# wanzysky/SlenderObjDet

Hardware: AMD Instinct MI355X
Metric: training img/sec FCOS R50-FPN 1333x800 (higher is better)
Workload: dtype bf16; 1 GPU; FCOS R50-FPN (FCOSV2, giou, center-sampling 1.5), fwd+bwd+SGD, synthetic 1333x800 padded to 800x1344 (BASELINE.json configs[1]); global_batch=16, parallelism=dp1

## Files before the change

### slenderobjdet_amd/csrc/conv_args.h

```cpp
#pragma once
#include "common.h"
#include "../../include/slender_hip.h"
#include <stdlib.h>

namespace sodconv {

enum { MODE_FWD = 0, MODE_DGRAD = 1 };
enum {
  F_BIAS = 1, F_RELU = 2, F_RES = 4, F_RES_UP2 = 8, F_MASK = 16,
  F_WBITS = 64,
  F_MASKBITS = 128,
  F_GNSTATS = 32,
  F_REVERSE = 1024,
  F_RES_EVEN = 512,
};
constexpr int MAXLEV = SOD_CONV_MAX_LEVELS;

struct LevelGeo {
  const void* src;
  void* dst;
  const void* res;
  const void* mask;
  void* bits;
  float* gn_sum;
// ... 46 lines not shown
template <int LPR>
__device__ __forceinline__ void gn_acc_finish(GnAcc& g, uint32_t pa, uint32_t pb, uint32_t P, const FastDiv& div_hw, float* sums, int G, int grp,
                                              bool qok, int lane) {
  if (pa >= P) return;
  if (pb >= P) pb = P - 1;
  const int na = (int)fd_div(pa, div_hw), nb = (int)fd_div(pb, div_hw);
  if (na == nb) {
    float s = (g.n >= 0) ? g.s : 0.f, ss = (g.n >= 0) ? g.ss : 0.f;
#pragma unroll
    for (int o = LPR; o < 64; o <<= 1) { s += __shfl_xor(s, o, 64); ss += __shfl_xor(ss, o, 64); }
    if (lane < LPR && qok) {
      atomicAdd(sums + ((size_t)na * G + grp) * 2, s);
      atomicAdd(sums + ((size_t)na * G + grp) * 2 + 1, ss);
    }
  } else if (qok) {
    gn_acc_flush(g, sums, G, grp);
  }
}

enum ConvTile { TILE_16x256, TILE_64x256, TILE_64x256_K32, TILE_128x128, TILE_128x128_K32 };
int launch_conv128(const ConvArgs& a, int mode, bool out_f32, ConvTile tile, bool generic, hipStream_t st, int* variant);

bool conv256_supported(const ConvArgs& a, int mode);
int launch_conv256(const ConvArgs& a, int mode, bool out_f32, int max_pt_tiles, hipStream_t st);

bool pw_supported(const ConvArgs& a, int mode, bool out_f32, int cus);
int launch_pw(const ConvArgs& a, int mode, hipStream_t st);

bool ws3_supported(const ConvArgs& a, int mode, bool out_f32, int cus, bool any_size);
int launch_ws3(const ConvArgs& a, int mode, hipStream_t st);

struct WLevel {
  const void* dy;
  const void* x;
  uint32_t dy_bytes, x_bytes;
  int Hx, Wx, Ho, Wo, P;
  int v0;
  int dy_img_stride, x_img_stride;
  FastDiv div_hw, div_w;
};

struct WgradArgs {
  WLevel lev[MAXLEV];
  int nlev;
  float* dw;
  const float* qscale;
  int dbg_plain_store;
// ... 31 lines not shown
```

### slenderobjdet_amd/csrc/conv_dispatch.hip

```cpp
#include "conv_args.h"
#include <stdlib.h>
#include <atomic>
#include <algorithm>

using namespace sodconv;

int device_cus() {
  static const int cus = [] {
    int dev = 0, n = 0;
    if (hipGetDevice(&dev) != hipSuccess || hipDeviceGetAttribute(&n, hipDeviceAttributeMultiprocessorCount, dev) != hipSuccess || n <= 0) n = 256;
    return n;
  }();
  return cus;
}

namespace {

thread_local int g_last_variant = 0;
thread_local int g_conv_reverse = 0;

struct ConvKnobs {
  int conv256 = -1;
  int pw = -1;
  int ws3 = -1;
  int wgrad256 = 1;
  int wgrad9 = 1;
  int wgrad9_min_kt = 24;
  int wgrad_variant = -1;
};
ConvKnobs& knobs() {
  const auto env = [](const char* name, int dflt) { const char* e = getenv(name); return e ? atoi(e) : dflt; };
  static ConvKnobs k = [&] {
    ConvKnobs k0;
    k0.wgrad256 = env("SOD_WGRAD256", k0.wgrad256);
    k0.wgrad9 = env("SOD_WGRAD9", k0.wgrad9);
    k0.wgrad9_min_kt = env("SOD_WGRAD9_MIN_KT", k0.wgrad9_min_kt);
    return k0;
  }();
  if (k.conv256 < 0) k.conv256 = env("SOD_CONV256", 1);
  if (k.pw < 0) k.pw = env("SOD_CONV_PW", 1);
  if (k.ws3 < 0) k.ws3 = env("SOD_CONV_WS3", 1);
  return k;
}

struct ConvProf {
  hipEvent_t* ev = nullptr;
  int* variant = nullptr;
  int* mode = nullptr;
  float* frac = nullptr;
  int cap = 0;
  std::atomic<int> n{0};
  std::atomic<int> on{0};
};
ConvProf g_prof;
thread_local int g_prof_depth = 0;
inline int prof_begin(hipStream_t st) {
  ConvProf& p = g_prof;
  if (!p.on.load(std::memory_order_relaxed) || g_prof_depth) return -1;
  const int i = p.n.fetch_add(1);
  if (i >= p.cap) { p.n.store(p.cap); return -1; }
  (void)hipEventRecord(p.ev[2 * i], st);
  return i;
// ... 20 lines not shown
  if (a.cwin) {
    if (generic || a.nlev != 1 || (a.Nout & 127)) return SOD_EARG;
    return conv128(TILE_128x128);
  }
  const ConvKnobs& k = knobs();
  const int cus = device_cus();
  if (k.pw && pw_supported(a, mode, out_f32, cus)) {
    g_last_variant = 7001;
    return timed(st, 7001, 1.f, mode, [&] { return launch_pw(a, mode, st); });
  }
  if (k.ws3 && ws3_supported(a, mode, out_f32, cus, k.ws3 == 2)) {
    g_last_variant = 7003;
    return timed(st, 7003, 1.f, mode, [&] { return launch_ws3(a, mode, st); });
  }
  bool any_start = false;
  for (int l = 0; l < a.nlev; ++l) any_start |= a.lev[l].pstart != 0;
  if (k.conv256 && !any_start && !(a.flags & (F_WBITS | F_MASKBITS)) && conv256_supported(a, mode)) {
    const int nq = (a.Nout + 255) / 256;
    long long pt256 = 0;
    for (int l = 0; l < a.nlev; ++l) pt256 += (a.lev[l].P + 255) / 256;
    const long long b256 = pt256 * nq;
    const auto conv256 = [&](int max_pt_tiles, float frac) {
      g_last_variant = 256;
      return timed(st, 256, frac, mode, [&] { return launch_conv256(a, mode, out_f32, max_pt_tiles, st); });
    };
    if (k.conv256 == 2) return conv256(0, 1.f);
    constexpr int min_rounds = 1, min_k = 1024;
    if (a.Nout >= 256 && ((a.Nout & 255) == 0 || a.Nout >= 512) && a.Kred >= min_k && b256 >= (long long)min_rounds * cus) {
      const long long full = b256 / cus * cus, rem = b256 - full;
      if (rem == 0 || rem * 2 >= (long long)cus || (full / nq) * nq != full) return conv256(0, 1.f);
      int main_pt = (int)(full / nq);
      long long ptot = 0;
      for (int l = 0; l < a.nlev; ++l) ptot += a.lev[l].P;
      int rc = conv256(main_pt, (float)((double)main_pt * 256.0 / (double)ptot));
      if (rc) return rc;
      ConvArgs tail = a;
      for (int l = 0; l < tail.nlev; ++l) {
        const int tl = (tail.lev[l].P + 255) / 256;
        if (main_pt >= tl) { tail.lev[l].pstart = tail.lev[l].P; main_pt -= tl; }
        else { tail.lev[l].pstart = main_pt * 256; main_pt = 0; }
      }
      ++g_prof_depth;
      rc = dispatch_conv(tail, mode, out_f32, st);
      --g_prof_depth;
      g_last_variant = 256;
      return rc;
    }
// ... 419 lines not shown
  return SOD_OK;
}

extern "C" int sod_conv_set_wgrad_variant(int variant) {
  if (variant < -1) return SOD_EARG;
  knobs().wgrad_variant = variant;
  return SOD_OK;
}

extern "C" int sod_conv_set_ws3(int mode) {
  if (mode < -1 || mode > 2) return SOD_EARG;
  knobs().ws3 = mode;
  return SOD_OK;
}

extern "C" int sod_conv_set_pw(int on) {
  if (on < -1 || on > 1) return SOD_EARG;
  knobs().pw = on;
  return SOD_OK;
}

extern "C" int sod_conv_set_tile256(int mode) {
  if (mode < -1 || mode > 2) return SOD_EARG;
  knobs().conv256 = mode;
  return SOD_OK;
}
```

### slenderobjdet_amd/csrc/conv_igemm256.hip

```cpp
#include "conv_args.h"
#include <stdlib.h>
#include <type_traits>

namespace sodconv {
namespace {

constexpr int ROWB = 128;
constexpr int UNIT = 128 * ROWB;
constexpr int BUF = 4 * UNIT;
constexpr int LDS_BYTES = 2 * BUF;
constexpr int E16_PITCH = 256;

template <int SA, int SB, int KS>
__device__ __forceinline__ void mma_half(f32x4_t (&acc)[8][4], const bf16x8_t (&af)[4][2], const bf16x8_t (&bf)[2][2]) {
#pragma unroll
  for (int i = 0; i < 4; ++i)
#pragma unroll
    for (int j = 0; j < 2; ++j)
      acc[SA * 4 + i][SB * 2 + j] = __builtin_amdgcn_mfma_f32_16x16x32_bf16(af[i][KS], bf[j][KS], acc[SA * 4 + i][SB * 2 + j], 0, 0, 0);
}

#define SOD256_SB __builtin_amdgcn_sched_barrier(0);
#define SOD256_PHASE(SA, SB, BFR, STAGE)                                  \
  asm volatile("s_waitcnt vmcnt(6)" ::: "memory");                        \
  __builtin_amdgcn_s_barrier();                                           \
  asm volatile("s_waitcnt lgkmcnt(0)" ::: "memory");                      \
  SOD256_SB                                                               \
  __builtin_amdgcn_s_setprio(1);                                          \
  mma_half<SA, SB, 0>(acc, af, BFR);                                      \
  SOD256_SB                                                               \
  STAGE;                                                                  \
  SOD256_SB                                                               \
  mma_half<SA, SB, 1>(acc, af, BFR);                                      \
  __builtin_amdgcn_s_setprio(0);                                          \
  __builtin_amdgcn_s_barrier();

template <int MODE, bool OUT_F32>
__global__ __launch_bounds__(512, 2) void conv_igemm256_kernel(const ConvArgs a) {
  extern __shared__ __attribute__((aligned(16))) char smem[];
  const int tid = threadIdx.x, lane = tid & 63;
  const int wave = __builtin_amdgcn_readfirstlane(tid >> 6);
  const int wr = wave >> 2, wc = wave & 3;
  uint32_t bid = xcd_remap(blockIdx.x, gridDim.x);
  if (a.flags & F_REVERSE) bid = gridDim.x - 1 - bid;
  const int qt = bid % a.nq_tiles;
  int pt = bid / a.nq_tiles;
  int lv = 0;
#pragma unroll
  for (int i = 1; i < MAXLEV; ++i)
    if (i < a.nlev && pt >= a.lev[i].tile0) lv = i;
  const LevelGeo& g = a.lev[lv];
  pt -= g.tile0;
  const int q0 = qt * 256, p0 = pt * 256;
  const int gP = g.P, gHs = g.Hs, gWs = g.Ws;
  const int T = a.T;

  auto wrsrc = __builtin_amdgcn_make_buffer_rsrc(const_cast<void*>(a.w), 0, a.w_bytes, 0x00020000);
  auto xrsrc = __builtin_amdgcn_make_buffer_rsrc(const_cast<void*>(g.src), 0, g.src_bytes, 0x00020000);

  const int srow = lane >> 3, spos = lane & 7;
  const int sswz = (lane >> 4) | ((wave & 1) << 2);
  const int schunk = spos ^ sswz;
  uint32_t wbase[2][2], rowbase[2][2], tapmask[2][2];
#pragma unroll
  for (int u = 0; u < 2; ++u)
#pragma unroll
    for (int j = 0; j < 2; ++j) {
      const int L = (j * 8 + wave) * 8 + srow;
      const int q = q0 + (L >> 6) * 128 + u * 64 + (L & 63);
      wbase[u][j] = (q < a.Nout) ? ((uint32_t)q * (uint32_t)a.Kred + (uint32_t)schunk * 8u) * 2u : SOD_OOB;
    }
  const uint32_t rs_mul = a.div_rs.mul, rs_shr = a.div_rs.shr, rs_d = a.div_rs.d;
  const int aCred = a.Cred;
  const bool pitched = a.Cpitch < a.Cred;
  auto stage_a = [&](int u, int kt) {
    char* dst = smem + (kt & 1) * BUF + u * UNIT + wave * 1024;
    const bool live = kt < T;
    const uint32_t kk = live ? (uint32_t)kt : 0u;
    const uint32_t cc = (__umulhi(kk, rs_mul) + kk) >> rs_shr;
    const uint32_t woff = ((kk - cc * rs_d) * (uint32_t)aCred + cc * 64u) * 2u;
    const uint32_t dead = live ? 0u : SOD_OOB;
#pragma unroll
    for (int j = 0; j < 2; ++j) {
      const uint32_t voff = (wbase[u][j] + woff) | dead;
      __builtin_amdgcn_raw_ptr_buffer_load_lds(wrsrc, SOD_LDS(dst + j * 8192), 16, voff, 0, 0, 0);
    }
  };
  stage_a(0, 0); stage_a(1, 0);
#pragma unroll
  for (int u = 0; u < 2; ++u)
#pragma unroll
    for (int j = 0; j < 2; ++j) {
      const int L = (j * 8 + wave) * 8 + srow;
      const uint32_t p = (uint32_t)(p0 + (L >> 5) * 64 + u * 32 + (L & 31));
      uint32_t m = 0, rb = 0;
      if (p < (uint32_t)gP) {
        const uint32_t n = fd_div(p, g.div_hw);
        const uint32_t rem = p - n * g.div_hw.d;
        const uint32_t ph = fd_div(rem, g.div_w);
        const uint32_t pw = rem - ph * g.div_w.d;
        int xh, xw;
        if (MODE == MODE_FWD) { xh = (int)ph * a.stride - a.pad; xw = (int)pw * a.stride - a.pad; }
        else                  { xh = (int)ph + a.pad;            xw = (int)pw + a.pad; }
        rb = (n * (uint32_t)g.src_img_stride + ((uint32_t)xh * (uint32_t)gWs + (uint32_t)xw) * (uint32_t)a.Cpitch + (uint32_t)schunk * 8u) * 2u;
        uint32_t colbits = 0;
        for (int s2 = 0; s2 < a.S; ++s2) {
          const int w = (MODE == MODE_FWD) ? xw + s2 * a.dil : xw - s2 * a.dil;
          colbits |= (uint32_t)((unsigned)w < (unsigned)gWs) << s2;
        }
        for (int r = 0; r < a.R; ++r) {
          const int h = (MODE == MODE_FWD) ? xh + r * a.dil : xh - r * a.dil;
          if ((unsigned)h < (unsigned)gHs) m |= colbits << (r * a.S);
        }
      }
      rowbase[u][j] = rb; tapmask[u][j] = m;
    }
  const int tap_sign = (MODE == MODE_FWD) ? 1 : -1;

  const uint32_t s_mul = a.div_s.mul, s_shr = a.div_s.shr;
  const int aS = a.S, row_step = a.dil * gWs * a.Cpitch * 2 * tap_sign, col_step = a.dil * a.Cpitch * 2 * tap_sign;

  auto stage_b = [&](int u, int kt) {
    char* dst = smem + (kt & 1) * BUF + (2 + u) * UNIT + wave * 1024;
    const bool live = kt < T;
    const uint32_t kk = live ? (uint32_t)kt : 0u;
    const uint32_t cc = (__umulhi(kk, rs_mul) + kk) >> rs_shr;
    const uint32_t tap = kk - cc * rs_d;
    const int c0 = (int)cc * 128;
    const int r = (int)((__umulhi(tap, s_mul) + tap) >> s_shr);
    const int s2 = (int)tap - r * aS;
    const uint32_t tapoff = (uint32_t)(r * row_step + s2 * col_step + c0);
    const uint32_t tbit = live ? tap : 31u;
    const bool cin = !pitched || ((int)cc * 64 + schunk * 8 < a.Cpitch);
#pragma unroll
    for (int j = 0; j < 2; ++j) {
      const uint32_t voff = (((tapmask[u][j] >> tbit) & 1u) && cin) ? rowbase[u][j] + tapoff : SOD_OOB;
      __builtin_amdgcn_raw_ptr_buffer_load_lds(xrsrc, SOD_LDS(dst + j * 8192), 16, voff, 0, 0, 0);
    }
  };

  const int fr = lane & 15, fg = lane >> 4;
  uint32_t aoff[4], boff[2];
#pragma unroll
  for (int i = 0; i < 4; ++i) {
    const int L = wr * 64 + i * 16 + fr;
    aoff[i] = L * ROWB + ((fg ^ ((L >> 1) & 7)) << 4);
  }
#pragma unroll
  for (int j = 0; j < 2; ++j) {
    const int L = wc * 32 + j * 16 + fr;
    boff[j] = 2 * UNIT + L * ROWB + ((fg ^ ((L >> 1) & 7)) << 4);
  }

  f32x4_t acc[8][4];
#pragma unroll
  for (int i = 0; i < 8; ++i)
#pragma unroll
    for (int j = 0; j < 4; ++j) acc[i][j] = f32x4_t{0.f, 0.f, 0.f, 0.f};
  bf16x8_t af[4][2], bf0[2][2], bf1[2][2];

  auto read_a = [&](const char* buf, int s) {
#pragma unroll
    for (int i = 0; i < 4; ++i)
#pragma unroll
      for (int ks = 0; ks < 2; ++ks) af[i][ks] = *reinterpret_cast<const bf16x8_t*>(buf + s * UNIT + (aoff[i] ^ (ks << 6)));
  };
  auto read_b = [&](const char* buf, int s, bf16x8_t (&bfr)[2][2]) {
#pragma unroll
    for (int j = 0; j < 2; ++j)
#pragma unroll
      for (int ks = 0; ks < 2; ++ks) bfr[j][ks] = *reinterpret_cast<const bf16x8_t*>(buf + s * UNIT + (boff[j] ^ (ks << 6)));
  };

  stage_b(0, 0); stage_b(1, 0);
  stage_a(0, 1); stage_b(0, 1);
  asm volatile("s_waitcnt vmcnt(4)" ::: "memory");
  __builtin_amdgcn_s_barrier();
  if (wr == 1) __builtin_amdgcn_s_barrier();

  for (int k = 0; k < T; ++k) {
    const char* cur = smem + (k & 1) * BUF;
    read_b(cur, 0, bf0);
    read_a(cur, 0);
    SOD256_PHASE(0, 0, bf0, stage_b(1, k + 1))
    read_b(cur, 1, bf1);
    SOD256_PHASE(0, 1, bf1, stage_a(1, k + 1))
    read_a(cur, 1);
    SOD256_PHASE(1, 1, bf1, stage_a(0, k + 2))
    SOD256_PHASE(1, 0, bf0, stage_b(0, k + 2))
  }
  if (wr == 0) __builtin_amdgcn_s_barrier();
  asm volatile("s_waitcnt vmcnt(0)" ::: "memory");
  __builtin_amdgcn_s_barrier();

  const int Nout = a.Nout;
  constexpr int QW = 128;
  constexpr int EROWB = QW * 4 + 16;
  constexpr int EPL = OUT_F32 ? 4 : 8;
  constexpr int LPR = QW / EPL;
  constexpr int ERPP = 64 / LPR;
  char* wl = smem + wave * (16 * EROWB);
  const int erow = lane / LPR, eq = (lane % LPR) * EPL;
  const int q = q0 + wr * QW + eq;
  constexpr int NP = 16 / ERPP;
  using RV = typename std::conditional<EPL == 8, bf16x8_t, bf16x4_t>::type;
  const bool qok = q < Nout;
  float bv[EPL];
#pragma unroll
  for (int e = 0; e < EPL; ++e) bv[e] = 0.f;
  if ((a.flags & F_BIAS) && qok) {
#pragma unroll
    for (int e = 0; e < EPL; e += 4) {
      const f32x4_t b = *reinterpret_cast<const f32x4_t*>(a.bias + q + e);
      bv[e] = b[0]; bv[e + 1] = b[1]; bv[e + 2] = b[2]; bv[e + 3] = b[3];
    }
  }
  GnAcc ga{0.f, 0.f, -1};
  if constexpr (!OUT_F32) {
    if (!(a.flags & (F_RES | F_RES_UP2))) {
      char* w16 = smem + wave * (64 * E16_PITCH);
#pragma unroll
      for (int i = 0; i < 8; ++i) {
        f32x4_t b4 = {0.f, 0.f, 0.f, 0.f};
        const int qa = q0 + wr * QW + i * 16 + fg * 4;
        if ((a.flags & F_BIAS) && qa < Nout) b4 = *reinterpret_cast<const f32x4_t*>(a.bias + qa);
#pragma unroll
        for (int jj = 0; jj < 4; ++jj) {
          f32x4_t v = acc[i][jj] + b4;
          if (a.flags & F_RELU) { v[0] = fmaxf(v[0], 0.f); v[1] = fmaxf(v[1], 0.f); v[2] = fmaxf(v[2], 0.f); v[3] = fmaxf(v[3], 0.f); }
          bf16x4_t o = {(__bf16)v[0], (__bf16)v[1], (__bf16)v[2], (__bf16)v[3]};
          *reinterpret_cast<bf16x4_t*>(w16 + (jj * 16 + fr) * E16_PITCH + (((i * 4 + fg) ^ (2 * fr)) << 3)) = o;
        }
      }
#pragma unroll
      for (int jj = 0; jj < 4; ++jj) {
        const uint32_t pfirst = (uint32_t)(p0 + wc * 64 + jj * 16 + erow);
        const uint32_t pc0 = pfirst < (uint32_t)gP ? pfirst : 0u;
        uint32_t n_run = fd_div(pc0, g.div_hw);
        uint32_t rem_run = pc0 - n_run * g.div_hw.d;
#pragma unroll
        for (int k = 0; k < NP; ++k) {
          const uint32_t p = pfirst + (uint32_t)(k * ERPP);
          const bool okk = (p < (uint32_t)gP) && qok;
          const uint32_t n = n_run, rem = rem_run;
          rem_run += (uint32_t)ERPP;
          while (rem_run >= g.div_hw.d) { rem_run -= g.div_hw.d; ++n_run; }
          if (okk) {
            const size_t drow = (size_t)n * g.dst_img_stride + (size_t)rem * Nout;
            bf16x8_t o = *reinterpret_cast<const bf16x8_t*>(w16 + (jj * 16 + k * ERPP + erow) * E16_PITCH + (((eq >> 3) ^ (k * ERPP + erow)) << 4));
            if (a.flags & F_MASK) {
              const bf16x8_t mv = *reinterpret_cast<const bf16x8_t*>((const __bf16*)g.mask + drow + q);
#pragma unroll
              for (int e = 0; e < 8; ++e) o[e] = ((float)mv[e] > 0.f) ? o[e] : (__bf16)0.f;
            }
            sod_store16((__bf16*)g.dst + drow + q, o);
            if constexpr (MODE == MODE_FWD) { if (a.flags & F_GNSTATS) gn_acc_add(ga, (int)n, o, g.gn_sum, a.gn_G, q >> 3); }
          }
        }
      }
      if constexpr (MODE == MODE_FWD) {
        if (a.flags & F_GNSTATS)
          gn_acc_finish<LPR>(ga, (uint32_t)(p0 + wc * 64), (uint32_t)(p0 + wc * 64 + 63), (uint32_t)gP, g.div_hw, g.gn_sum, a.gn_G, q >> 3, qok, lane);
      }
      return;
    }
  }
#pragma unroll
  for (int jj = 0; jj < 4; ++jj) {
    RV resv[NP], maskv[NP];
    size_t drow[NP];
    bool ok[NP];
    int nimg[NP];
    const uint32_t pfirst = (uint32_t)(p0 + wc * 64 + jj * 16 + erow);
    const uint32_t pc0 = pfirst < (uint32_t)gP ? pfirst : 0u;
    uint32_t n_run = fd_div(pc0, g.div_hw);
    uint32_t rem_run = pc0 - n_run * g.div_hw.d;
#pragma unroll
    for (int k = 0; k < NP; ++k) {
      const uint32_t p = pfirst + (uint32_t)(k * ERPP);
      ok[k] = (p < (uint32_t)gP) && qok;
      drow[k] = 0;
      const uint32_t n = n_run, rem = rem_run;
      rem_run += (uint32_t)ERPP;
      while (rem_run >= g.div_hw.d) { rem_run -= g.div_hw.d; ++n_run; }
      if (ok[k]) {
        nimg[k] = (int)n;
        drow[k] = (size_t)n * g.dst_img_stride + (size_t)rem * Nout;
        if (a.flags & (F_RES | F_RES_UP2)) {
          size_t res_row;
          if (a.flags & F_RES_UP2) {
            const uint32_t ph = fd_div(rem, g.div_w);
            const uint32_t pw = rem - ph * g.div_w.d;
            res_row = (size_t)n * g.res_img_stride + (size_t)((ph >> 1) * (g.Wp >> 1) + (pw >> 1)) * Nout;
          } else {
            res_row = (size_t)n * g.res_img_stride + (size_t)rem * Nout;
          }
          resv[k] = *reinterpret_cast<const RV*>((const __bf16*)g.res + res_row + q);
        }
        if (a.flags & F_MASK) maskv[k] = *reinterpret_cast<const RV*>((const __bf16*)g.mask + drow[k] + q);
      }
    }
#pragma unroll
    for (int i = 0; i < 8; ++i)
      *reinterpret_cast<f32x4_t*>(wl + fr * EROWB + (i * 16 + fg * 4) * 4) = acc[i][jj];
#pragma unroll
    for (int k = 0; k < NP; ++k) {
      const int row = k * ERPP + erow;
      if (ok[k]) {
        float v[EPL];
#pragma unroll
        for (int e = 0; e < EPL; e += 4) {
          const f32x4_t t4 = *reinterpret_cast<const f32x4_t*>(wl + row * EROWB + (eq + e) * 4);
          v[e] = t4[0]; v[e + 1] = t4[1]; v[e + 2] = t4[2]; v[e + 3] = t4[3];
        }
        if (a.flags & F_BIAS) {
#pragma unroll
          for (int e = 0; e < EPL; ++e) v[e] += bv[e];
        }
        if (a.flags & (F_RES | F_RES_UP2)) {
#pragma unroll
          for (int e = 0; e < EPL; ++e) v[e] += (float)resv[k][e];
        }
        if (a.flags & F_RELU) {
#pragma unroll
          for (int e = 0; e < EPL; ++e) v[e] = fmaxf(v[e], 0.f);
        }
        if (a.flags & F_MASK) {
#pragma unroll
          for (int e = 0; e < EPL; ++e) v[e] = ((float)maskv[k][e] > 0.f) ? v[e] : 0.f;
        }
        if constexpr (OUT_F32) {
          sod_store16((float*)g.dst + drow[k] + q, f32x4_t{v[0], v[1], v[2], v[3]});
        } else {
          bf16x8_t o;
#pragma unroll
          for (int e = 0; e < 8; ++e) o[e] = (__bf16)v[e];
          sod_store16((__bf16*)g.dst + drow[k] + q, o);
          if constexpr (MODE == MODE_FWD) { if (a.flags & F_GNSTATS) gn_acc_add(ga, nimg[k], o, g.gn_sum, a.gn_G, q >> 3); }
        }
      }
    }
  }
  if constexpr (!OUT_F32 && MODE == MODE_FWD) {
    if (a.flags & F_GNSTATS)
      gn_acc_finish<LPR>(ga, (uint32_t)(p0 + wc * 64), (uint32_t)(p0 + wc * 64 + 63), (uint32_t)gP, g.div_hw, g.gn_sum, a.gn_G, q >> 3, qok, lane);
  }
}

template <int MODE, bool OUT_F32>
int launch256(const ConvArgs& a0, int max_pt_tiles, hipStream_t st) {
  ConvArgs a = a0;
  a.T = a.Kred / 64;
  a.div_cpt = make_fastdiv((uint32_t)(a.Cred / 64));
  a.div_rs = make_fastdiv((uint32_t)(a.R * a.S));
  a.tap_inner = 1;
  a.nq_tiles = (a.Nout + 255) / 256;
  int tiles = 0;
  for (int l = 0; l < a.nlev; ++l) {
    a.lev[l].tile0 = tiles;
    tiles += (a.lev[l].P + 255) / 256;
  }
  a.np_tiles = (max_pt_tiles > 0 && max_pt_tiles < tiles) ? max_pt_tiles : tiles;
  constexpr auto kern = conv_igemm256_kernel<MODE, OUT_F32>;
  const hipError_t e = sod_max_dynamic_lds_once<kern>(LDS_BYTES);
  if (e != hipSuccess) return (int)e;
  SOD_LAUNCH(kern, dim3(a.nq_tiles * a.np_tiles), dim3(512), LDS_BYTES, st, a);
  SOD_CHECK_LAUNCH();
  return SOD_OK;
}

}

bool conv256_supported(const ConvArgs& a, int mode) {
  if ((a.Cred & 63) || (a.Nout & 7) || a.R * a.S > 31 || a.cwin) return false;
  if (mode == MODE_DGRAD && a.stride != 1) return false;
  return true;
}

int launch_conv256(const ConvArgs& a, int mode, bool out_f32, int max_pt_tiles, hipStream_t st) {
  if (!conv256_supported(a, mode)) return SOD_EARG;
  if (mode == MODE_FWD) return out_f32 ? launch256<MODE_FWD, true>(a, max_pt_tiles, st) : launch256<MODE_FWD, false>(a, max_pt_tiles, st);
  return out_f32 ? launch256<MODE_DGRAD, true>(a, max_pt_tiles, st) : launch256<MODE_DGRAD, false>(a, max_pt_tiles, st);
}

}
```

Before: 667.3 img/s.

## Make conv256 igemm kernel persistent with cross-tile prefetch of next tile

After: 660.0 img/s. 1.1% lower.

```diff
diff --git a/slenderobjdet_amd/csrc/conv_args.h b/slenderobjdet_amd/csrc/conv_args.h
--- a/slenderobjdet_amd/csrc/conv_args.h
+++ b/slenderobjdet_amd/csrc/conv_args.h
@@ -92,7 +92,7 @@
 int launch_conv128(const ConvArgs& a, int mode, bool out_f32, ConvTile tile, bool generic, hipStream_t st, int* variant);
 
 bool conv256_supported(const ConvArgs& a, int mode);
-int launch_conv256(const ConvArgs& a, int mode, bool out_f32, int max_pt_tiles, hipStream_t st);
+int launch_conv256(const ConvArgs& a, int mode, bool out_f32, int max_pt_tiles, int persist, hipStream_t st);
 
 bool pw_supported(const ConvArgs& a, int mode, bool out_f32, int cus);
 int launch_pw(const ConvArgs& a, int mode, hipStream_t st);
diff --git a/slenderobjdet_amd/csrc/conv_dispatch.hip b/slenderobjdet_amd/csrc/conv_dispatch.hip
--- a/slenderobjdet_amd/csrc/conv_dispatch.hip
+++ b/slenderobjdet_amd/csrc/conv_dispatch.hip
@@ -21,6 +21,7 @@
 
 struct ConvKnobs {
   int conv256 = -1;
+  int conv256_persist = -1;
   int pw = -1;
   int ws3 = -1;
   int wgrad256 = 1;
@@ -38,6 +39,7 @@
     return k0;
   }();
   if (k.conv256 < 0) k.conv256 = env("SOD_CONV256", 1);
+  if (k.conv256_persist < 0) k.conv256_persist = env("SOD_CONV256_PERSIST", 1) != 0;
   if (k.pw < 0) k.pw = env("SOD_CONV_PW", 1);
   if (k.ws3 < 0) k.ws3 = env("SOD_CONV_WS3", 1);
   return k;
@@ -104,7 +106,7 @@
     const long long b256 = pt256 * nq;
     const auto conv256 = [&](int max_pt_tiles, float frac) {
       g_last_variant = 256;
-      return timed(st, 256, frac, mode, [&] { return launch_conv256(a, mode, out_f32, max_pt_tiles, st); });
+      return timed(st, 256, frac, mode, [&] { return launch_conv256(a, mode, out_f32, max_pt_tiles, k.conv256_persist, st); });
     };
     if (k.conv256 == 2) return conv256(0, 1.f);
     constexpr int min_rounds = 1, min_k = 1024;
@@ -570,6 +572,8 @@
 
 extern "C" int sod_conv_set_tile256(int mode) {
   if (mode < -1 || mode > 2) return SOD_EARG;
-  knobs().conv256 = mode;
-  return SOD_OK;
-}
+  ConvKnobs& k = knobs();
+  k.conv256 = mode;
+  k.conv256_persist = -1;
+  return SOD_OK;
+}
diff --git a/slenderobjdet_amd/csrc/conv_igemm256.hip b/slenderobjdet_amd/csrc/conv_igemm256.hip
--- a/slenderobjdet_amd/csrc/conv_igemm256.hip
+++ b/slenderobjdet_amd/csrc/conv_igemm256.hip
@@ -41,60 +41,55 @@
   const int tid = threadIdx.x, lane = tid & 63;
   const int wave = __builtin_amdgcn_readfirstlane(tid >> 6);
   const int wr = wave >> 2, wc = wave & 3;
-  uint32_t bid = xcd_remap(blockIdx.x, gridDim.x);
-  if (a.flags & F_REVERSE) bid = gridDim.x - 1 - bid;
-  const int qt = bid % a.nq_tiles;
-  int pt = bid / a.nq_tiles;
-  int lv = 0;
-#pragma unroll
-  for (int i = 1; i < MAXLEV; ++i)
-    if (i < a.nlev && pt >= a.lev[i].tile0) lv = i;
-  const LevelGeo& g = a.lev[lv];
-  pt -= g.tile0;
-  const int q0 = qt * 256, p0 = pt * 256;
-  const int gP = g.P, gHs = g.Hs, gWs = g.Ws;
   const int T = a.T;
+#define SOD256_WAIT_VM(N) do { asm volatile("" ::: "memory"); __builtin_amdgcn_s_waitcnt(0x0F70 | ((N) & 15) | (((N) >> 4) << 14)); asm volatile("" ::: "memory"); } while (0)
+#define SOD256_ARGS() (*[]() { auto p = (const __attribute__((address_space(4))) char*)__builtin_amdgcn_kernarg_segment_ptr(); asm volatile("" : "+s"(p)); return (const ConvArgs*)p; }())
+  const uint32_t ntiles = (uint32_t)a.nq_tiles * (uint32_t)a.np_tiles, gstride = gridDim.x;
+  auto tile_of = [&](const ConvArgs& a, uint32_t v, int& q0_, int& p0_, int& lv_) {
+    uint32_t bid = xcd_remap(v, ntiles);
+    if (a.flags & F_REVERSE) bid = ntiles - 1 - bid;
+    const int qt = bid % a.nq_tiles;
+    int pt = bid / a.nq_tiles;
+    int lv = 0;
+#pragma unroll
+    for (int i = 1; i < MAXLEV; ++i)
+      if (i < a.nlev && pt >= a.lev[i].tile0) lv = i;
+    pt -= a.lev[lv].tile0;
+    q0_ = qt * 256; p0_ = pt * 256; lv_ = lv;
+  };
 
   auto wrsrc = __builtin_amdgcn_make_buffer_rsrc(const_cast<void*>(a.w), 0, a.w_bytes, 0x00020000);
-  auto xrsrc = __builtin_amdgcn_make_buffer_rsrc(const_cast<void*>(g.src), 0, g.src_bytes, 0x00020000);
-
-  const int srow = lane >> 3, spos = lane & 7;
+
+  const int spos = lane & 7;
   const int sswz = (lane >> 4) | ((wave & 1) << 2);
   const int schunk = spos ^ sswz;
   uint32_t wbase[2][2], rowbase[2][2], tapmask[2][2];
-#pragma unroll
-  for (int u = 0; u < 2; ++u)
+  uint32_t wbase_n[2][2] = {{SOD_OOB, SOD_OOB}, {SOD_OOB, SOD_OOB}}, rowbase_n[2][2] = {{0, 0}, {0, 0}}, tapmask_n[2][2] = {{0, 0}, {0, 0}};
+  auto geo_w = [&](const ConvArgs& a, int q0_, uint32_t (&wb)[2][2]) {
+    int gl = lane;
+    asm volatile("" : "+v"(gl));
+    const int srow = gl >> 3, schunk = (gl & 7) ^ ((gl >> 4) | ((wave & 1) << 2));
+#pragma unroll
+    for (int u = 0; u < 2; ++u)
+#pragma unroll
+      for (int j = 0; j < 2; ++j) {
+        const int L = (j * 8 + wave) * 8 + srow;
+        const int q = q0_ + (L >> 6) * 128 + u * 64 + (L & 63);
+        wb[u][j] = (q < a.Nout) ? ((uint32_t)q * (uint32_t)a.Kred + (uint32_t)schunk * 8u) * 2u : SOD_OOB;
+      }
+  };
+  auto geo_p = [&](const ConvArgs& a, int u, int p0_, int lv_, uint32_t (&rbs)[2][2], uint32_t (&tms)[2][2]) {
+    const LevelGeo& g = a.lev[lv_];
+    const int gHs = g.Hs, gWs = g.Ws;
+    int gl = lane;
+    asm volatile("" : "+v"(gl));
+    const int srow = gl >> 3, schunk = (gl & 7) ^ ((gl >> 4) | ((wave & 1) << 2));
 #pragma unroll
     for (int j = 0; j < 2; ++j) {
       const int L = (j * 8 + wave) * 8 + srow;
-      const int q = q0 + (L >> 6) * 128 + u * 64 + (L & 63);
-      wbase[u][j] = (q < a.Nout) ? ((uint32_t)q * (uint32_t)a.Kred + (uint32_t)schunk * 8u) * 2u : SOD_OOB;
-    }
-  const uint32_t rs_mul = a.div_rs.mul, rs_shr = a.div_rs.shr, rs_d = a.div_rs.d;
-  const int aCred = a.Cred;
-  const bool pitched = a.Cpitch < a.Cred;
-  auto stage_a = [&](int u, int kt) {
-    char* dst = smem + (kt & 1) * BUF + u * UNIT + wave * 1024;
-    const bool live = kt < T;
-    const uint32_t kk = live ? (uint32_t)kt : 0u;
-    const uint32_t cc = (__umulhi(kk, rs_mul) + kk) >> rs_shr;
-    const uint32_t woff = ((kk - cc * rs_d) * (uint32_t)aCred + cc * 64u) * 2u;
-    const uint32_t dead = live ? 0u : SOD_OOB;
-#pragma unroll
-    for (int j = 0; j < 2; ++j) {
-      const uint32_t voff = (wbase[u][j] + woff) | dead;
-      __builtin_amdgcn_raw_ptr_buffer_load_lds(wrsrc, SOD_LDS(dst + j * 8192), 16, voff, 0, 0, 0);
-    }
-  };
-  stage_a(0, 0); stage_a(1, 0);
-#pragma unroll
-  for (int u = 0; u < 2; ++u)
-#pragma unroll
-    for (int j = 0; j < 2; ++j) {
-      const int L = (j * 8 + wave) * 8 + srow;
-      const uint32_t p = (uint32_t)(p0 + (L >> 5) * 64 + u * 32 + (L & 31));
+      const uint32_t p = (uint32_t)(p0_ + (L >> 5) * 64 + u * 32 + (L & 31));
       uint32_t m = 0, rb = 0;
-      if (p < (uint32_t)gP) {
+      if (p < (uint32_t)g.P) {
         const uint32_t n = fd_div(p, g.div_hw);
         const uint32_t rem = p - n * g.div_hw.d;
         const uint32_t ph = fd_div(rem, g.div_w);
@@ -113,15 +108,39 @@
           if ((unsigned)h < (unsigned)gHs) m |= colbits << (r * a.S);
         }
       }
-      rowbase[u][j] = rb; tapmask[u][j] = m;
-    }
+      rbs[u][j] = rb; tms[u][j] = m;
+    }
+  };
   const int tap_sign = (MODE == MODE_FWD) ? 1 : -1;
 
+  const uint32_t rs_mul = a.div_rs.mul, rs_shr = a.div_rs.shr, rs_d = a.div_rs.d;
   const uint32_t s_mul = a.div_s.mul, s_shr = a.div_s.shr;
-  const int aS = a.S, row_step = a.dil * gWs * a.Cpitch * 2 * tap_sign, col_step = a.dil * a.Cpitch * 2 * tap_sign;
-
+  const int aCred = a.Cred;
+  const bool pitched = a.Cpitch < a.Cred;
+  const int aS = a.S, col_step = a.dil * a.Cpitch * 2 * tap_sign;
+
+  int q0, p0, lv, q0_n = 0, p0_n = 0, lv_n = 0;
+  uint32_t xlo = 0, xhi = 0, xbytes = 0, xlo_n = 0, xhi_n = 0, xbytes_n = 0;
+  auto xrsrc = __builtin_amdgcn_make_buffer_rsrc((void*)nullptr, 0, 0, 0x00020000);
+  int row_step, row_step_n = 0;
+  int par = 0;
+  bool pipe = false;
+
+  auto stage_a = [&](int u, int kt) {
+    char* dst = smem + ((par + kt) & 1) * BUF + u * UNIT + wave * 1024;
+    const bool live = kt < T;
+    const uint32_t kk = live ? (uint32_t)kt : 0u;
+    const uint32_t cc = (__umulhi(kk, rs_mul) + kk) >> rs_shr;
+    const uint32_t woff = ((kk - cc * rs_d) * (uint32_t)aCred + cc * 64u) * 2u;
+    const uint32_t dead = live ? 0u : SOD_OOB;
+#pragma unroll
+    for (int j = 0; j < 2; ++j) {
+      const uint32_t voff = (wbase[u][j] + woff) | dead;
+      __builtin_amdgcn_raw_ptr_buffer_load_lds(wrsrc, SOD_LDS(dst + j * 8192), 16, voff, 0, 0, 0);
+    }
+  };
   auto stage_b = [&](int u, int kt) {
-    char* dst = smem + (kt & 1) * BUF + (2 + u) * UNIT + wave * 1024;
+    char* dst = smem + ((par + kt) & 1) * BUF + (2 + u) * UNIT + wave * 1024;
     const bool live = kt < T;
     const uint32_t kk = live ? (uint32_t)kt : 0u;
     const uint32_t cc = (__umulhi(kk, rs_mul) + kk) >> rs_shr;
@@ -138,6 +157,31 @@
       __builtin_amdgcn_raw_ptr_buffer_load_lds(xrsrc, SOD_LDS(dst + j * 8192), 16, voff, 0, 0, 0);
     }
   };
+  auto stage_a_next = [&](int u, int kk) {
+    char* dst = smem + ((par + T + kk) & 1) * BUF + u * UNIT + wave * 1024;
+    const uint32_t cc = (__umulhi((uint32_t)kk, rs_mul) + (uint32_t)kk) >> rs_shr;
+    const uint32_t woff = (((uint32_t)kk - cc * rs_d) * (uint32_t)aCred + cc * 64u) * 2u;
+#pragma unroll
+    for (int j = 0; j < 2; ++j)
+      __builtin_amdgcn_raw_ptr_buffer_load_lds(wrsrc, SOD_LDS(dst + j * 8192), 16, wbase_n[u][j] + woff, 0, 0, 0);
+  };
+  auto stage_b_next = [&](int u, int kk) {
+    char* dst = smem + ((par + T + kk) & 1) * BUF + (2 + u) * UNIT + wave * 1024;
+    const uint32_t cc = (__umulhi((uint32_t)kk, rs_mul) + (uint32_t)kk) >> rs_shr;
+    const uint32_t tap = (uint32_t)kk - cc * rs_d;
+    const int c0 = (int)cc * 128;
+    const int r = (int)((__umulhi(tap, s_mul) + tap) >> s_shr);
+    const int s2 = (int)tap - r * aS;
+    const uint32_t tapoff = (uint32_t)(r * row_step_n + s2 * col_step + c0);
+    const bool cin = !pitched || ((int)cc * 64 + schunk * 8 < a.Cpitch);
+    auto xrsrc_n = __builtin_amdgcn_make_buffer_rsrc(reinterpret_cast<void*>(((uint64_t)(uint32_t)__builtin_amdgcn_readfirstlane(xhi_n) << 32) | (uint32_t)__builtin_amdgcn_readfirstlane(xlo_n)), 0,
+                                                     __builtin_amdgcn_readfirstlane(xbytes_n), 0x00020000);
+#pragma unroll
+    for (int j = 0; j < 2; ++j) {
+      const uint32_t voff = (((tapmask_n[u][j] >> tap) & 1u) && cin) ? rowbase_n[u][j] + tapoff : SOD_OOB;
+      __builtin_amdgcn_raw_ptr_buffer_load_lds(xrsrc_n, SOD_LDS(dst + j * 8192), 16, voff, 0, 0, 0);
+    }
+  };
 
   const int fr = lane & 15, fg = lane >> 4;
   uint32_t aoff[4], boff[2];
@@ -153,10 +197,6 @@
   }
 
   f32x4_t acc[8][4];
-#pragma unroll
-  for (int i = 0; i < 8; ++i)
-#pragma unroll
-    for (int j = 0; j < 4; ++j) acc[i][j] = f32x4_t{0.f, 0.f, 0.f, 0.f};
   bf16x8_t af[4][2], bf0[2][2], bf1[2][2];
 
   auto read_a = [&](const char* buf, int s) {
@@ -172,183 +212,298 @@
       for (int ks = 0; ks < 2; ++ks) bfr[j][ks] = *reinterpret_cast<const bf16x8_t*>(buf + s * UNIT + (boff[j] ^ (ks << 6)));
   };
 
-  stage_b(0, 0); stage_b(1, 0);
-  stage_a(0, 1); stage_b(0, 1);
-  asm volatile("s_waitcnt vmcnt(4)" ::: "memory");
-  __builtin_amdgcn_s_barrier();
-  if (wr == 1) __builtin_amdgcn_s_barrier();
-
-  for (int k = 0; k < T; ++k) {
-    const char* cur = smem + (k & 1) * BUF;
-    read_b(cur, 0, bf0);
-    read_a(cur, 0);
-    SOD256_PHASE(0, 0, bf0, stage_b(1, k + 1))
-    read_b(cur, 1, bf1);
-    SOD256_PHASE(0, 1, bf1, stage_a(1, k + 1))
-    read_a(cur, 1);
-    SOD256_PHASE(1, 1, bf1, stage_a(0, k + 2))
-    SOD256_PHASE(1, 0, bf0, stage_b(0, k + 2))
-  }
-  if (wr == 0) __builtin_amdgcn_s_barrier();
-  asm volatile("s_waitcnt vmcnt(0)" ::: "memory");
-  __builtin_amdgcn_s_barrier();
-
-  const int Nout = a.Nout;
   constexpr int QW = 128;
   constexpr int EROWB = QW * 4 + 16;
   constexpr int EPL = OUT_F32 ? 4 : 8;
   constexpr int LPR = QW / EPL;
   constexpr int ERPP = 64 / LPR;
-  char* wl = smem + wave * (16 * EROWB);
-  const int erow = lane / LPR, eq = (lane % LPR) * EPL;
-  const int q = q0 + wr * QW + eq;
   constexpr int NP = 16 / ERPP;
   using RV = typename std::conditional<EPL == 8, bf16x8_t, bf16x4_t>::type;
-  const bool qok = q < Nout;
-  float bv[EPL];
-#pragma unroll
-  for (int e = 0; e < EPL; ++e) bv[e] = 0.f;
-  if ((a.flags & F_BIAS) && qok) {
-#pragma unroll
-    for (int e = 0; e < EPL; e += 4) {
-      const f32x4_t b = *reinterpret_cast<const f32x4_t*>(a.bias + q + e);
-      bv[e] = b[0]; bv[e + 1] = b[1]; bv[e + 2] = b[2]; bv[e + 3] = b[3];
-    }
-  }
-  GnAcc ga{0.f, 0.f, -1};
-  if constexpr (!OUT_F32) {
-    if (!(a.flags & (F_RES | F_RES_UP2))) {
-      char* w16 = smem + wave * (64 * E16_PITCH);
-#pragma unroll
-      for (int i = 0; i < 8; ++i) {
-        f32x4_t b4 = {0.f, 0.f, 0.f, 0.f};
-        const int qa = q0 + wr * QW + i * 16 + fg * 4;
-        if ((a.flags & F_BIAS) && qa < Nout) b4 = *reinterpret_cast<const f32x4_t*>(a.bias + qa);
-#pragma unroll
-        for (int jj = 0; jj < 4; ++jj) {
-          f32x4_t v = acc[i][jj] + b4;
-          if (a.flags & F_RELU) { v[0] = fmaxf(v[0], 0.f); v[1] = fmaxf(v[1], 0.f); v[2] = fmaxf(v[2], 0.f); v[3] = fmaxf(v[3], 0.f); }
-          bf16x4_t o = {(__bf16)v[0], (__bf16)v[1], (__bf16)v[2], (__bf16)v[3]};
-          *reinterpret_cast<bf16x4_t*>(w16 + (jj * 16 + fr) * E16_PITCH + (((i * 4 + fg) ^ (2 * fr)) << 3)) = o;
+
+  const bool bf16_whole = !OUT_F32 && !(a.flags & (F_RES | F_RES_UP2));
+  uint32_t vtile = blockIdx.x;
+  bool staged = false;
+  tile_of(a, vtile, q0, p0, lv);
+  for (;;) {
+    const uint32_t vnext = vtile + gstride;
+    const bool has_next = vnext < ntiles;
+    pipe = has_next && T >= 3 && bf16_whole;
+    if (!staged) {
+      const ConvArgs& at = SOD256_ARGS();
+      xlo = (uint32_t)(uintptr_t)at.lev[lv].src; xhi = (uint32_t)((uintptr_t)at.lev[lv].src >> 32); xbytes = at.lev[lv].src_bytes;
+    }
+    xrsrc = __builtin_amdgcn_make_buffer_rsrc(reinterpret_cast<void*>(((uint64_t)(uint32_t)__builtin_amdgcn_readfirstlane(xhi) << 32) | (uint32_t)__builtin_amdgcn_readfirstlane(xlo)), 0,
+                                              __builtin_amdgcn_readfirstlane(xbytes), 0x00020000);
+    if (!staged) {
+      const ConvArgs& at = SOD256_ARGS();
+      row_step = at.dil * at.lev[lv].Ws * at.Cpitch * 2 * tap_sign;
+      geo_w(at, q0, wbase);
+      stage_a(0, 0); stage_a(1, 0);
+      geo_p(at, 0, p0, lv, rowbase, tapmask);
+      geo_p(at, 1, p0, lv, rowbase, tapmask);
+      stage_b(0, 0); stage_b(1, 0);
+      stage_a(0, 1); stage_b(0, 1);
+      SOD256_WAIT_VM(4);
+      __builtin_amdgcn_s_barrier();
+      if (wr == 1) __builtin_amdgcn_s_barrier();
+    }
+#pragma unroll
+    for (int i = 0; i < 8; ++i)
+#pragma unroll
+      for (int j = 0; j < 4; ++j) acc[i][j] = f32x4_t{0.f, 0.f, 0.f, 0.f};
+
+#define SOD256_KTILE(K, S0, S1, S2, S3)                                                  \
+    {                                                                                      \
+      const char* cur = smem + ((par + (K)) & 1) * BUF;                                    \
+                                                           \
+      read_b(cur, 0, bf0);                                                                 \
+      read_a(cur, 0);                                                                      \
+      SOD256_PHASE(0, 0, bf0, S0)                                                          \
+                                                           \
+      read_b(cur, 1, bf1);                                                                 \
+      SOD256_PHASE(0, 1, bf1, S1)                                                          \
+                                                           \
+      read_a(cur, 1);                                                                      \
+      SOD256_PHASE(1, 1, bf1, S2)                                                          \
+                                    \
+      SOD256_PHASE(1, 0, bf0, S3)                                                          \
+    }
+    const int kmain = pipe ? T - 2 : T;
+    for (int k = 0; k < kmain; ++k) SOD256_KTILE(k, stage_b(1, k + 1), stage_a(1, k + 1), stage_a(0, k + 2), stage_b(0, k + 2))
+    if (pipe) {
+      auto geo0 = [&]() {
+        const ConvArgs& an = SOD256_ARGS();
+        tile_of(an, vnext, q0_n, p0_n, lv_n);
+        const LevelGeo& gn = an.lev[lv_n];
+        xlo_n = __builtin_amdgcn_readfirstlane((uint32_t)(uintptr_t)gn.src); xhi_n = __builtin_amdgcn_readfirstlane((uint32_t)((uintptr_t)gn.src >> 32));
+        xbytes_n = __builtin_amdgcn_readfirstlane(gn.src_bytes);
+        row_step_n = an.dil * gn.Ws * an.Cpitch * 2 * tap_sign;
+        geo_w(an, q0_n, wbase_n);
+      };
+      SOD256_KTILE(T - 2, (geo0(), stage_b(1, T - 1)), (geo_p(SOD256_ARGS(), 0, p0_n, lv_n, rowbase_n, tapmask_n), stage_a(1, T - 1)),
+                   (geo_p(SOD256_ARGS(), 1, p0_n, lv_n, rowbase_n, tapmask_n), stage_a_next(0, 0)), stage_b_next(0, 0))
+      SOD256_KTILE(T - 1, stage_b_next(1, 0), stage_a_next(1, 0), (void)0, (void)0)
+    }
+    if (wr == 0) __builtin_amdgcn_s_barrier();
+    if (!pipe) {
+      SOD256_WAIT_VM(0);
+      __builtin_amdgcn_s_barrier();
+    }
+    int elane = lane, ewave = wave;
+    asm volatile("" : "+v"(elane), "+s"(ewave));
+    const int efr = elane & 15, efg = elane >> 4, ewr = ewave >> 2, ewc = ewave & 3;
+    const int erow = elane / LPR, eq = (elane % LPR) * EPL;
+    char* const ebuf = smem + ((par + T - 1) & 1) * BUF + ewave * 8192;
+    auto after_lds = [&]() {
+      asm volatile("s_waitcnt lgkmcnt(0)" ::: "memory");
+      __builtin_amdgcn_s_barrier();
+      if (pipe) { stage_a_next(0, 1); stage_b_next(0, 1); }
+    };
+
+    const ConvArgs& ae = SOD256_ARGS();
+    const LevelGeo& g = ae.lev[lv];
+    const int Nout = ae.Nout, eflags = ae.flags;
+    const int q = q0 + ewr * QW + eq;
+    const bool qok = q < Nout;
+    const int gP = g.P;
+    GnAcc ga{0.f, 0.f, -1};
+    const bool wave_full = bf16_whole && (uint32_t)(p0 + ewc * 64 + 63) < (uint32_t)gP && q0 + ewr * QW + QW <= Nout;
+    if constexpr (!OUT_F32) {
+      if (bf16_whole) {
+        f32x4_t b4s[8];
+#pragma unroll
+        for (int i = 0; i < 8; ++i) b4s[i] = f32x4_t{0.f, 0.f, 0.f, 0.f};
+        if (eflags & F_BIAS) {
+#pragma unroll
+          for (int i = 0; i < 8; ++i) {
+            const int qa = q0 + ewr * QW + i * 16 + efg * 4;
+            b4s[i] = *reinterpret_cast<const f32x4_t*>(ae.bias + (qa < Nout ? qa : Nout - 4));
+          }
+#pragma unroll
+          for (int i = 0; i < 8; ++i) {
+            const int qa = q0 + ewr * QW + i * 16 + efg * 4;
+            if (qa >= Nout) b4s[i] = f32x4_t{0.f, 0.f, 0.f, 0.f};
+          }
+        }
+#pragma unroll
+        for (int i = 0; i < 8; ++i) {
+          const f32x4_t b4 = b4s[i];
+#pragma unroll
+          for (int jj = 0; jj < 4; ++jj) {
+            f32x4_t v = acc[i][jj] + b4;
+            if (eflags & F_RELU) { v[0] = fmaxf(v[0], 0.f); v[1] = fmaxf(v[1], 0.f); v[2] = fmaxf(v[2], 0.f); v[3] = fmaxf(v[3], 0.f); }
+            acc[i][jj] = v;
+          }
+        }
+#pragma unroll
+        for (int h = 0; h < 2; ++h) {
+#pragma unroll
+          for (int i = 0; i < 8; ++i)
+#pragma unroll
+            for (int j2 = 0; j2 < 2; ++j2) {
+              const f32x4_t v = acc[i][h * 2 + j2];
+              bf16x4_t o = {(__bf16)v[0], (__bf16)v[1], (__bf16)v[2], (__bf16)v[3]};
+              *reinterpret_cast<bf16x4_t*>(ebuf + (j2 * 16 + efr) * E16_PITCH + (((i * 4 + efg) ^ (2 * efr)) << 3)) = o;
+            }
+          bf16x8_t ov[2][NP];
+          uint32_t drow[2][NP];
+          int nimg[2][NP];
+          bool okk[2][NP];
+#pragma unroll
+          for (int j2 = 0; j2 < 2; ++j2) {
+            const uint32_t pfirst = (uint32_t)(p0 + ewc * 64 + (h * 2 + j2) * 16 + erow);
+            const uint32_t pc0 = pfirst < (uint32_t)gP ? pfirst : 0u;
+            uint32_t n_run = fd_div(pc0, g.div_hw);
+            uint32_t rem_run = pc0 - n_run * g.div_hw.d;
+#pragma unroll
+            for (int k = 0; k < NP; ++k) {
+              const uint32_t p = pfirst + (uint32_t)(k * ERPP);
+              okk[j2][k] = (p < (uint32_t)gP) && qok;
+              const uint32_t n = n_run, rem = rem_run;
+              rem_run += (uint32_t)ERPP;
+              while (rem_run >= g.div_hw.d) { rem_run -= g.div_hw.d; ++n_run; }
+              nimg[j2][k] = (int)n;
+              drow[j2][k] = n * (uint32_t)g.dst_img_stride + rem * (uint32_t)Nout;
+              bf16x8_t o = *reinterpret_cast<const bf16x8_t*>(ebuf + (j2 * 16 + k * ERPP + erow) * E16_PITCH + (((eq >> 3) ^ (k * ERPP + erow)) << 4));
+              if ((eflags & F_MASK) && okk[j2][k]) {
+                const bf16x8_t mv = *reinterpret_cast<const bf16x8_t*>((const __bf16*)g.mask + drow[j2][k] + q);
+#pragma unroll
+                for (int e = 0; e < 8; ++e) o[e] = ((float)mv[e] > 0.f) ? o[e] : (__bf16)0.f;
+              }
+              ov[j2][k] = o;
+            }
+          }
+          if (h == 1) after_lds();
+#pragma unroll
+          for (int j2 = 0; j2 < 2; ++j2)
+#pragma unroll
+            for (int k = 0; k < NP; ++k)
+              if (okk[j2][k]) {
+                sod_store16((__bf16*)g.dst + drow[j2][k] + q, ov[j2][k]);
+                if constexpr (MODE == MODE_FWD) { if (eflags & F_GNSTATS) gn_acc_add(ga, nimg[j2][k], ov[j2][k], g.gn_sum, ae.gn_G, q >> 3); }
+              }
         }
       }
+    }
+    if (!bf16_whole) {
+      char* const wl = smem + ewave * (16 * EROWB);
+      float bv[EPL];
+#pragma unroll
+      for (int e = 0; e < EPL; ++e) bv[e] = 0.f;
+      if ((eflags & F_BIAS) && qok) {
+#pragma unroll
+        for (int e = 0; e < EPL; e += 4) {
+          const f32x4_t b = *reinterpret_cast<const f32x4_t*>(ae.bias + q + e);
+          bv[e] = b[0]; bv[e + 1] = b[1]; bv[e + 2] = b[2]; bv[e + 3] = b[3];
+        }
+      }
 #pragma unroll
       for (int jj = 0; jj < 4; ++jj) {
-        const uint32_t pfirst = (uint32_t)(p0 + wc * 64 + jj * 16 + erow);
+        RV resv[NP] = {}, maskv[NP] = {};
+        size_t drow[NP];
+        bool ok[NP];
+        int nimg[NP] = {};
+        const uint32_t pfirst = (uint32_t)(p0 + ewc * 64 + jj * 16 + erow);
         const uint32_t pc0 = pfirst < (uint32_t)gP ? pfirst : 0u;
         uint32_t n_run = fd_div(pc0, g.div_hw);
         uint32_t rem_run = pc0 - n_run * g.div_hw.d;
 #pragma unroll
         for (int k = 0; k < NP; ++k) {
           const uint32_t p = pfirst + (uint32_t)(k * ERPP);
-          const bool okk = (p < (uint32_t)gP) && qok;
+          ok[k] = (p < (uint32_t)gP) && qok;
+          drow[k] = 0;
           const uint32_t n = n_run, rem = rem_run;
           rem_run += (uint32_t)ERPP;
           while (rem_run >= g.div_hw.d) { rem_run -= g.div_hw.d; ++n_run; }
-          if (okk) {
-            const size_t drow = (size_t)n * g.dst_img_stride + (size_t)rem * Nout;
-            bf16x8_t o = *reinterpret_cast<const bf16x8_t*>(w16 + (jj * 16 + k * ERPP + erow) * E16_PITCH + (((eq >> 3) ^ (k * ERPP + erow)) << 4));
-            if (a.flags & F_MASK) {
-              const bf16x8_t mv = *reinterpret_cast<const bf16x8_t*>((const __bf16*)g.mask + drow + q);
-#pragma unroll
-              for (int e = 0; e < 8; ++e) o[e] = ((float)mv[e] > 0.f) ? o[e] : (__bf16)0.f;
-            }
-            sod_store16((__bf16*)g.dst + drow + q, o);
-            if constexpr (MODE == MODE_FWD) { if (a.flags & F_GNSTATS) gn_acc_add(ga, (int)n, o, g.gn_sum, a.gn_G, q >> 3); }
+          if (ok[k]) {
+            nimg[k] = (int)n;
+            drow[k] = (size_t)n * g.dst_img_stride + (size_t)rem * Nout;
+            if (eflags & (F_RES | F_RES_UP2)) {
+              size_t res_row;
+              if (eflags & F_RES_UP2) {
+                const uint32_t ph = fd_div(rem, g.div_w);
+                const uint32_t pw = rem - ph * g.div_w.d;
+                res_row = (size_t)n * g.res_img_stride + (size_t)((ph >> 1) * (g.Wp >> 1) + (pw >> 1)) * Nout;
+              } else {
+                res_row = (size_t)n * g.res_img_stride + (size_t)rem * Nout;
+              }
+              resv[k] = *reinterpret_cast<const RV*>((const __bf16*)g.res + res_row + q);
+            }
+            if (eflags & F_MASK) maskv[k] = *reinterpret_cast<const RV*>((const __bf16*)g.mask + drow[k] + q);
           }
         }
+#pragma unroll
+        for (int i = 0; i < 8; ++i)
+          *reinterpret_cast<f32x4_t*>(wl + efr * EROWB + (i * 16 + efg * 4) * 4) = acc[i][jj];
+#pragma unroll
+        for (int k = 0; k < NP; ++k) {
+          const int row = k * ERPP + erow;
+          if (ok[k]) {
+            float v[EPL];
+#pragma unroll
+            for (int e = 0; e < EPL; e += 4) {
+              const f32x4_t t4 = *reinterpret_cast<const f32x4_t*>(wl + row * EROWB + (eq + e) * 4);
+              v[e] = t4[0]; v[e + 1] = t4[1]; v[e + 2] = t4[2]; v[e + 3] = t4[3];
+            }
+            if (eflags & F_BIAS) {
+#pragma unroll
+              for (int e = 0; e < EPL; ++e) v[e] += bv[e];
+            }
+            if (eflags & (F_RES | F_RES_UP2)) {
+#pragma unroll
+              for (int e = 0; e < EPL; ++e) v[e] += (float)resv[k][e];
+            }
+            if (eflags & F_RELU) {
+#pragma unroll
+              for (int e = 0; e < EPL; ++e) v[e] = fmaxf(v[e], 0.f);
+            }
+            if (eflags & F_MASK) {
+#pragma unroll
+              for (int e = 0; e < EPL; ++e) v[e] = ((float)maskv[k][e] > 0.f) ? v[e] : 0.f;
+            }
+            if constexpr (OUT_F32) {
+              sod_store16((float*)g.dst + drow[k] + q, f32x4_t{v[0], v[1], v[2], v[3]});
+            } else {
+              bf16x8_t o;
+#pragma unroll
+              for (int e = 0; e < 8; ++e) o[e] = (__bf16)v[e];
+              sod_store16((__bf16*)g.dst + drow[k] + q, o);
+              if constexpr (MODE == MODE_FWD) { if (eflags & F_GNSTATS) gn_acc_add(ga, nimg[k], o, g.gn_sum, ae.gn_G, q >> 3); }
+            }
+          }
+        }
       }
-      if constexpr (MODE == MODE_FWD) {
-        if (a.flags & F_GNSTATS)
-          gn_acc_finish<LPR>(ga, (uint32_t)(p0 + wc * 64), (uint32_t)(p0 + wc * 64 + 63), (uint32_t)gP, g.div_hw, g.gn_sum, a.gn_G, q >> 3, qok, lane);
-      }
-      return;
+      SOD256_WAIT_VM(0);
+      after_lds();
+    }
+    if constexpr (!OUT_F32 && MODE == MODE_FWD) {
+      if (eflags & F_GNSTATS)
+        gn_acc_finish<LPR>(ga, (uint32_t)(p0 + ewc * 64), (uint32_t)(p0 + ewc * 64 + 63), (uint32_t)gP, g.div_hw, g.gn_sum, ae.gn_G, q >> 3, qok, elane);
+    }
+    if (!has_next) break;
+
+    par = (par + T) & 1;
+    vtile = vnext;
+    if (pipe) {
+#pragma unroll
+      for (int u = 0; u < 2; ++u)
+#pragma unroll
+        for (int j = 0; j < 2; ++j) { wbase[u][j] = wbase_n[u][j]; rowbase[u][j] = rowbase_n[u][j]; tapmask[u][j] = tapmask_n[u][j]; }
+      q0 = q0_n; p0 = p0_n; lv = lv_n;
+      xlo = xlo_n; xhi = xhi_n; xbytes = xbytes_n; row_step = row_step_n;
+      if (wave_full) SOD256_WAIT_VM(20); else SOD256_WAIT_VM(4);
+      __builtin_amdgcn_s_barrier();
+      if (wr == 1) __builtin_amdgcn_s_barrier();
+      staged = true;
+    } else {
+      tile_of(SOD256_ARGS(), vtile, q0, p0, lv);
+      staged = false;
     }
   }
-#pragma unroll
-  for (int jj = 0; jj < 4; ++jj) {
-    RV resv[NP], maskv[NP];
-    size_t drow[NP];
-    bool ok[NP];
-    int nimg[NP];
-    const uint32_t pfirst = (uint32_t)(p0 + wc * 64 + jj * 16 + erow);
-    const uint32_t pc0 = pfirst < (uint32_t)gP ? pfirst : 0u;
-    uint32_t n_run = fd_div(pc0, g.div_hw);
-    uint32_t rem_run = pc0 - n_run * g.div_hw.d;
-#pragma unroll
-    for (int k = 0; k < NP; ++k) {
-      const uint32_t p = pfirst + (uint32_t)(k * ERPP);
-      ok[k] = (p < (uint32_t)gP) && qok;
-      drow[k] = 0;
-      const uint32_t n = n_run, rem = rem_run;
-      rem_run += (uint32_t)ERPP;
-      while (rem_run >= g.div_hw.d) { rem_run -= g.div_hw.d; ++n_run; }
-      if (ok[k]) {
-        nimg[k] = (int)n;
-        drow[k] = (size_t)n * g.dst_img_stride + (size_t)rem * Nout;
-        if (a.flags & (F_RES | F_RES_UP2)) {
-          size_t res_row;
-          if (a.flags & F_RES_UP2) {
-            const uint32_t ph = fd_div(rem, g.div_w);
-            const uint32_t pw = rem - ph * g.div_w.d;
-            res_row = (size_t)n * g.res_img_stride + (size_t)((ph >> 1) * (g.Wp >> 1) + (pw >> 1)) * Nout;
-          } else {
-            res_row = (size_t)n * g.res_img_stride + (size_t)rem * Nout;
-          }
-          resv[k] = *reinterpret_cast<const RV*>((const __bf16*)g.res + res_row + q);
-        }
-        if (a.flags & F_MASK) maskv[k] = *reinterpret_cast<const RV*>((const __bf16*)g.mask + drow[k] + q);
-      }
-    }
-#pragma unroll
-    for (int i = 0; i < 8; ++i)
-      *reinterpret_cast<f32x4_t*>(wl + fr * EROWB + (i * 16 + fg * 4) * 4) = acc[i][jj];
-#pragma unroll
-    for (int k = 0; k < NP; ++k) {
-      const int row = k * ERPP + erow;
-      if (ok[k]) {
-        float v[EPL];
-#pragma unroll
-        for (int e = 0; e < EPL; e += 4) {
-          const f32x4_t t4 = *reinterpret_cast<const f32x4_t*>(wl + row * EROWB + (eq + e) * 4);
-          v[e] = t4[0]; v[e + 1] = t4[1]; v[e + 2] = t4[2]; v[e + 3] = t4[3];
-        }
-        if (a.flags & F_BIAS) {
-#pragma unroll
-          for (int e = 0; e < EPL; ++e) v[e] += bv[e];
-        }
-        if (a.flags & (F_RES | F_RES_UP2)) {
-#pragma unroll
-          for (int e = 0; e < EPL; ++e) v[e] += (float)resv[k][e];
-        }
-        if (a.flags & F_RELU) {
-#pragma unroll
-          for (int e = 0; e < EPL; ++e) v[e] = fmaxf(v[e], 0.f);
-        }
-        if (a.flags & F_MASK) {
-#pragma unroll
-          for (int e = 0; e < EPL; ++e) v[e] = ((float)maskv[k][e] > 0.f) ? v[e] : 0.f;
-        }
-        if constexpr (OUT_F32) {
-          sod_store16((float*)g.dst + drow[k] + q, f32x4_t{v[0], v[1], v[2], v[3]});
-        } else {
-          bf16x8_t o;
-#pragma unroll
-          for (int e = 0; e < 8; ++e) o[e] = (__bf16)v[e];
-          sod_store16((__bf16*)g.dst + drow[k] + q, o);
-          if constexpr (MODE == MODE_FWD) { if (a.flags & F_GNSTATS) gn_acc_add(ga, nimg[k], o, g.gn_sum, a.gn_G, q >> 3); }
-        }
-      }
-    }
-  }
-  if constexpr (!OUT_F32 && MODE == MODE_FWD) {
-    if (a.flags & F_GNSTATS)
-      gn_acc_finish<LPR>(ga, (uint32_t)(p0 + wc * 64), (uint32_t)(p0 + wc * 64 + 63), (uint32_t)gP, g.div_hw, g.gn_sum, a.gn_G, q >> 3, qok, lane);
-  }
 }
 
 template <int MODE, bool OUT_F32>
-int launch256(const ConvArgs& a0, int max_pt_tiles, hipStream_t st) {
+int launch256(const ConvArgs& a0, int max_pt_tiles, int persist, hipStream_t st) {
   ConvArgs a = a0;
   a.T = a.Kred / 64;
   a.div_cpt = make_fastdiv((uint32_t)(a.Cred / 64));
@@ -364,7 +519,10 @@
   constexpr auto kern = conv_igemm256_kernel<MODE, OUT_F32>;
   const hipError_t e = sod_max_dynamic_lds_once<kern>(LDS_BYTES);
   if (e != hipSuccess) return (int)e;
-  SOD_LAUNCH(kern, dim3(a.nq_tiles * a.np_tiles), dim3(512), LDS_BYTES, st, a);
+  int grid = a.nq_tiles * a.np_tiles;
+  const int cus = device_cus() & ~7;
+  if (persist && cus > 0 && grid > cus) grid = cus;
+  SOD_LAUNCH(kern, dim3(grid), dim3(512), LDS_BYTES, st, a);
   SOD_CHECK_LAUNCH();
   return SOD_OK;
 }
@@ -377,10 +535,10 @@
   return true;
 }
 
-int launch_conv256(const ConvArgs& a, int mode, bool out_f32, int max_pt_tiles, hipStream_t st) {
+int launch_conv256(const ConvArgs& a, int mode, bool out_f32, int max_pt_tiles, int persist, hipStream_t st) {
   if (!conv256_supported(a, mode)) return SOD_EARG;
-  if (mode == MODE_FWD) return out_f32 ? launch256<MODE_FWD, true>(a, max_pt_tiles, st) : launch256<MODE_FWD, false>(a, max_pt_tiles, st);
-  return out_f32 ? launch256<MODE_DGRAD, true>(a, max_pt_tiles, st) : launch256<MODE_DGRAD, false>(a, max_pt_tiles, st);
-}
-
-}
+  if (mode == MODE_FWD) return out_f32 ? launch256<MODE_FWD, true>(a, max_pt_tiles, persist, st) : launch256<MODE_FWD, false>(a, max_pt_tiles, persist, st);
+  return out_f32 ? launch256<MODE_DGRAD, true>(a, max_pt_tiles, persist, st) : launch256<MODE_DGRAD, false>(a, max_pt_tiles, persist, st);
+}
+
+}
```
